# Prasaya/brax

Measured on AMD Instinct MI355X. Metric: env-steps/sec (Ant, 4096 envs/GPU), higher is better.
Workload: dtype f32

## Files before the change

brax_amd/csrc/pbd_eval.hip:

```cpp
#define BX_TU_FAST
#include <hip/hip_runtime.h>
#include <stdint.h>

#include "pbd_dispatch.h"
#include "pbd_kernels.hip"
#include "pbd_launch.h"

namespace bx {

template <int L, int MODE, int F, int M, int EK = EK_ANY>
__global__ void __launch_bounds__(L > 64 ? L : 64) BX_STEP_ATTR
env_eval_policy_kernel(EnvArgs A, PolArgs Q, EvalArgs V) {
  env_step_body<L, MODE, F, M, EK, true, false, true, true>(A, Q, V);
}
template <int L, int MODE, int F, int M, int EK = EK_ANY>
__global__ void __launch_bounds__(L > 64 ? L : 64) __attribute__((amdgpu_waves_per_eu(2)))
env_eval_policy_wide_kernel(EnvArgs A, PolArgs Q, EvalArgs V) {
  env_step_body<L, MODE, F, M, EK, true, false, true, true>(A, Q, V);
}

BX_ENV_FAMILY(EvalPolicyFamily, FAM_EVAL_POLICY, env_eval_policy_kernel, env_eval_policy_wide_kernel)
hipError_t launch_env_eval_policy(int L, int feat, int gw, int tpb, int64_t n_envs, size_t lds,
                                  hipStream_t s, const EnvArgs& a, const PolArgs& q,
                                  const EvalArgs& v, int fold) {
  return launch_env_family<EvalPolicyFamily>(L, feat, gw, tpb, n_envs, lds, s, fold, a, q, v);
}

}
```

brax_amd/csrc/pbd_features.h:

```cpp
#pragma once
#if defined(__HIPCC__)
#include <hip/hip_runtime.h>
#endif

namespace bx {

enum { F_SPH = 1, F_ANGLE = 2, F_CC = 4, F_TW = 8, F_FORCE = 16, F_ALL = 31 };
enum { F_G1 = 32 };
enum { F_X = 64, F_GEN = F_ALL | F_X };
enum { F_JH = 128 };
enum { F_R2 = 256 };
enum { F_C16 = 512 };
enum { F_R2G = 1024 };
enum { F_CCO = 2048 };
enum { F_LEAN = F_CC | F_TW };

constexpr bool cb_feat(int F) {
#if defined(BX_NO_CB)
  return false;
#else
  return (F & F_JH) != 0 && (F & F_G1) != 0 &&
         (F & (F_CC | F_TW | F_R2 | F_C16 | F_FORCE | F_SPH)) == 0;
#endif
}

#if defined(__HIPCC__)
template <int F, int M> __device__ __forceinline__ constexpr int cl_width() {
  return (F & F_C16) ? 16 : M;
}
template <int F> __device__ __forceinline__ bool is_rev(int type) {
  if constexpr ((F & F_SPH) == 0) return true; else return type == 1;
}
template <int F> __device__ __forceinline__ bool is_torque(int type) {
  if constexpr ((F & F_ANGLE) == 0) return true; else return type == 0;
}
template <int F> __device__ __forceinline__ bool is_plane(int fn) {
  if constexpr ((F & F_CCO) != 0) return false;
  else if constexpr ((F & F_CC) == 0) return true; else return fn == 0;
}
template <int F> __device__ __forceinline__ constexpr bool HALF() {
  return (F & F_CCO) != 0 && (F & F_R2G) != 0;
}
template <int F> __device__ __forceinline__ bool is_oneway(int ow) {
  if constexpr ((F & F_CCO) != 0) return false;
  else if constexpr ((F & F_TW) == 0) return true; else return ow != 0;
}
#endif

enum { LIM_G0 = 0, LIM_G1 = 2, LIM_G2 = 4, LIM_SLOTS = 6 };

enum { EK_ANY = 0, EK_ANT = 1, EK_HUM = 2, EK_CHEETAH = 3, EK_PUSHER = 4 };

enum { MODE_GLOBAL = 0, MODE_SINGLE = 1, MODE_LDS = 2, MODE_MULTI = 3 };

}
```

brax_amd/csrc/pbd_kernels.hip:

```cpp
#pragma once
#include <hip/hip_runtime.h>
#include <stdint.h>
#include <stdlib.h>
#include <string.h>

#include <type_traits>

#include "pbd_features.h"
#include "pbd_launch.h"
#include "pbd_layout.h"
#include "pbd_math.h"
#include "pbd_stamps.h"

namespace bx {

struct Cst {
  const uint32_t* __restrict__ w;
  __device__ __forceinline__ int i(int off) const { return (int)w[off]; }
  __device__ __forceinline__ float f(int off) const { return __uint_as_float(w[off]); }
  __device__ __forceinline__ v3 f3(int off) const { return mk(f(off), f(off + 1), f(off + 2)); }
};

struct BodyC {
  float mass;
// ... 469 lines not shown
}

__device__ __forceinline__ void seg_seg(v3 a0, v3 a1, v3 b0, v3 b1, v3& ba, v3& bb) {
  v3 da = a1 - a0;
  float la = safe_norm(da);
  la += 1e-6f * (float)(la == 0.f);
  da = da / la;
  float hla = la * 0.5f;
  v3 db = b1 - b0;
  float lb = safe_norm(db);
  lb += 1e-6f * (float)(lb == 0.f);
  db = db / lb;
  float hlb = lb * 0.5f;
  v3 am = a0 + da * hla, bm = b0 + db * hlb;
  v3 tr = am - bm;
  float dadb = dot(da, db), datr = dot(da, tr), dbtr = dot(db, tr);
  float den = 1.f - dadb * dadb;
  float ota = (-datr + dadb * dbtr) / (den + 1e-6f);
  float otb = dbtr + ota * dadb;
  float ta = clampf(ota, -hla, hla), tb = clampf(otb, -hlb, hlb);
  ba = am + da * ta;
  bb = bm + db * tb;
  v3 na, nb;
  float d1 = seg_point(a0, a1, bb, na);
  float d2 = seg_point(b0, b1, ba, nb);
  if (d1 < d2) ba = na; else bb = nb;
}

template <int F>
__device__ __forceinline__ void contact_gen(const RowC& R, const QP& a, const QP& b, v3& pos, v3& vel, v3& n,
                            float& pen) {
  if (is_plane<F>(R.fn)) {
  BX_IEEE_IN_CONTACT
    v3 e = a.pos + rotate(R.a_end, a.rot);
    n = rotate(mk(0.f, 0.f, 1.f), b.rot);
    pos = e - n * R.a_rad;
    vel = a.vel + cross(a.ang, pos - a.pos);
    pen = dot(b.pos - pos, n);
    return;
  }
  v3 pa = a.pos + rotate(R.a_pos, a.rot), ea = rotate(R.a_end, a.rot);
  v3 pb = b.pos + rotate(R.b_pos, b.rot), eb = rotate(R.b_end, b.rot);
  v3 a0 = pa + ea, a1 = pa - ea, b0 = pb + eb, b1 = pb - eb;
  v3 ba, bb;
  seg_seg(a0, a1, b0, b1, ba, bb);
  v3 pv = ba - bb;
  float dist = safe_norm(pv);
  n = pv / (1e-6f + dist);
  pen = R.a_rad + R.b_rad - dist + nan_of(dot(pv, pv));
  pos = (ba + bb) / 2.f;
  vel = (a.vel + cross(a.ang, pos - a.pos)) - (b.vel + cross(b.ang, pos - b.pos));
}


__device__ __forceinline__ float pdiv(float a, float b) { return (float)((double)a / (double)b); }

__device__ __noinline__ void heightmap_contact(const Cst& c, const BlobHdr& H, int o, const RowC& R,
                                               const QP& a, const QP& b, v3& pos, v3& vel, v3& n,
                                               float& pen) {
  const float cell = c.f(o + R_X);
  const int off = H.o_hm + c.i(o + R_HM_OFF), M = c.i(o + R_HM_M);
  v3 r = rotate(R.a_end, a.rot);
  pos = a.pos + r;
  vel = a.vel + cross(a.ang, r);
  v3 p = rotate(pos - b.pos, quat_inv(b.rot));
  float u = pdiv(p.x, cell), v = pdiv(p.y, cell);
  float fu = floorf(u), fv = floorf(v);
  int iu = (int)fu, iv = (int)fv;
  bool lower = ((u - fu) + (v - fv)) < 1.f;
  float mu = lower ? -1.f : 1.f;
  int tu[3] = {iu + (lower ? 0 : 1), iu + (lower ? 1 : 0), iu + (lower ? 0 : 1)};
  int tv[3] = {iv + (lower ? 0 : 1), iv + (lower ? 0 : 1), iv + (lower ? 1 : 0)};
  float hh[3];
#pragma unroll
  for (int k = 0; k < 3; k++) {
    int i = tu[k], j = -tv[k];
    i += i < 0 ? M : 0;
    j += j < 0 ? M : 0;
    i = i < 0 ? 0 : (i >= M ? M - 1 : i);
    j = j < 0 ? 0 : (j >= M ? M - 1 : j);
    hh[k] = c.f(off + i * M + j);
  }
  v3 raw = mk(mu * (hh[1] - hh[0]), mu * (hh[2] - hh[0]), cell);
  const float rn = safe_norm(raw);
  v3 n0 = mk(pdiv(raw.x, rn), pdiv(raw.y, rn), pdiv(raw.z, rn));
  v3 p0 = mk((float)tu[0] * cell, (float)tv[0] * cell, hh[0]);
  pen = dot(p0 - p, n0);
  n = rotate(n0, b.rot);
}

__device__ __noinline__ void clipped_contact(const Cst& c, int o, const RowC& R, const QP& a,
                                             const QP& b, v3& pos, v3& vel, v3& n, float& pen) {
  v3 e = a.pos + rotate(R.a_end, a.rot);
  v3 nb = rotate(c.f3(o + R_X), b.rot);
  float ndir = dot(a.pos, nb) > 0.f ? 1.f : -1.f;
  n = nb * ndir;
  pos = e - n * R.a_rad;
  vel = a.vel + cross(a.ang, pos - a.pos);
  v3 pt = rotate(c.f3(o + R_X + 9), b.rot) + b.pos;
  pen = dot(pt - pos, n);
  v3 nx = rotate(c.f3(o + R_X + 3), b.rot), ny = rotate(c.f3(o + R_X + 6), b.rot);
  const float hx = c.f(o + R_X + 12), hy = c.f(o + R_X + 13);
  v3 nn = n * ndir;
  v3 yn = cross(nn, nx), xn = -cross(nn, ny);
  bool front = dot(pos - (pt + nx * hx), xn) > 1e-6f;
  front |= dot(pos - (pt - nx * hx), -xn) > 1e-6f;
// ... 1707 lines not shown
    float c0 = 0.f;
#pragma unroll
    for (int k = 0; k < M; k++) {
      v3 v;
      q4 q;
      float f;
      ld_slot(cslot + (g.e[k] & 0xFFFFFF) * SLOT_STRIDE, v, q, f);
      if (!rot4) q = q4{0.f, q.w, q.x, q.y};
      a0 = a0 + v;
      r0 = r0 + q;
      c0 += f;
    }
    const float d0 = eps + c0;
    a = a0 / d0;
    r = q4{r0.w / d0, r0.x / d0, r0.y / d0, r0.z / d0};
    return;
  }
  const int g0 = g.e[0] >> 24;
  v3 a0 = mk(0.f, 0.f, 0.f), a1 = mk(0.f, 0.f, 0.f);
  q4 r0{0.f, 0.f, 0.f, 0.f}, r1{0.f, 0.f, 0.f, 0.f};
  float c0 = 0.f, c1 = 0.f;
#pragma unroll
  for (int k = 0; k < M; k++) {
    const float* s = cslot + (g.e[k] & 0xFFFFFF) * SLOT_STRIDE;
    float m0 = (g.e[k] >> 24) == g0 ? 1.f : 0.f;
    float m1 = 1.f - m0;
    v3 v;
    q4 q;
    float f;
    ld_slot(s, v, q, f);
    if (!rot4) q = q4{0.f, q.w, q.x, q.y};
    a0 = a0 + v * m0;
    a1 = a1 + v * m1;
    r0 = r0 + q * m0;
    r1 = r1 + q * m1;
    c0 += f * m0;
    c1 += f * m1;
  }
  float d0 = eps + c0, d1 = eps + c1;
  a = a0 / d0 + a1 / d1;
  r = q4{r0.w / d0 + r1.w / d1, r0.x / d0 + r1.x / d1, r0.y / d0 + r1.y / d1,
         r0.z / d0 + r1.z / d1};
}

__device__ __forceinline__ void own_contact(v3 v, q4 q, float f, float eps, v3& a, q4& r) {
  BX_IEEE_IN_CONTACT
  const v3 a0 = mk(0.f, 0.f, 0.f) + v;
  const q4 r0 = q4{0.f, 0.f, 0.f, 0.f} + q;
  const float d0 = eps + (0.f + f);
  a = a0 / d0;
  r = q4{r0.w / d0, r0.x / d0, r0.y / d0, r0.z / d0};
}

__device__ __forceinline__ void vproj(QP& q, v3 ppos, q4 prot, const BodyC& B, float h,
                                      bool bare = false, bool fast = false) {
  BX_IEEE_IN_BODY
  q4 nr = bare ? qnormalize_bare(q.rot) : qnormalize(q.rot, fast);
  const bool nd = !bare && !fast;
  q.vel = mul(nd ? ndiv3(q.pos - ppos, h) : (q.pos - ppos) / h, B.pm);
  q4 dq = quat_mul(nr, quat_inv(prot));
  v3 a = nd ? ndiv3(2.f * mk(dq.x, dq.y, dq.z), h) : 2.f * mk(dq.x, dq.y, dq.z) / h;
  float scl = dq.w >= 0.f ? 1.f : -1.f;
  q.ang = mul(mul(scl * B.rm, a), B.rm);
  q.rot = nr;
}

template <int L, int F, int M, bool FOLD = false, bool NOINFO = false, bool FULL = false>
__device__ void pbd_step_single(const Cst& c, const BlobHdr& H, const Env& E, int lane, bool valid,
                                const float* act, int aw, const Hoist<M, cl_width<F, M>()>& X,
                                v3& icv, v3& ica, v3& iaa) {
  static_assert(!FULL || ((F & F_JH) != 0 && L == 16), "FULL: the 16-lane joint halves");
  const bool hasB = FULL || X.hasB, hasJ = FULL || X.hasJ, hasA = FULL || X.hasA;
#ifdef BX_STAMPS
  unsigned long long st_acc[10] = {0, 0, 0, 0, 0, 0, 0, 0, 0, 0};
  unsigned long long st_last;
  asm volatile("s_memtime %0\n\ts_waitcnt lgkmcnt(0)" : "=s"(st_last)::"memory");
#endif
  const float h = H.h;
  const v3 g = mk(H.gx, H.gy, H.gz);
  constexpr bool JH = (F & F_JH) != 0;
  constexpr bool JLH = (F & F_SPH) == 0;
  const uint4* LIP = (F & F_SPH) != 0 ? E.jlim + lane : nullptr;
  const int jx = lane & 7;
  const bool child = (lane & 8) != 0;
  static_assert(!JH || (L == 16 && (F & F_SPH) == 0), "joint halves: revolute joints at 16 lanes");
  constexpr bool JB = FOLD && JH && (F & F_C16) == 0;
  constexpr bool CB = JB && cb_feat(F);
  const int bi = JB ? X.S.body : lane;
  float* myqp = E.qp + bi * QP_STRIDE;
  QP q;
  if (hasB) q = ldqp(myqp);
  if constexpr (JB) {
    if (lane < H.N) {
      const float* r = E.qp + lane * QP_STRIDE;
      const QP o = ldqp(r);
      st_slot(E.prev + lane * PREV_STRIDE, o.pos, o.rot, 0.f);
      st_rb(E.rb + lane * RB_STRIDE, o.pos, o.vel, o.ang);
      float* acc = E.acc + lane * ACC_STRIDE;
      st3(acc + ACC_ICV, mk(0.f, 0.f, 0.f));
      st3(acc + ACC_ICA, mk(0.f, 0.f, 0.f));
      st3(acc + ACC_IAA, mk(0.f, 0.f, 0.f));
    }
  }
  icv = mk(0.f, 0.f, 0.f);
  ica = mk(0.f, 0.f, 0.f);
  iaa = mk(0.f, 0.f, 0.f);
  float al[3] = {0.f, 0.f, 0.f};
  if (hasA && valid) {
#pragma unroll
    for (int l = 0; l < 3; l++) {
      int ai = X.A.idx[l];
      al[l] = act[take_idx(ai, aw)] * (ai >= 0 ? 1.f : 0.f);
    }
  }
  v3 fv = mk(0.f, 0.f, 0.f), fa = mk(0.f, 0.f, 0.f);
  if constexpr ((F & F_FORCE) != 0) {
    if (hasB) body_forces(c, H, lane, act, aw, valid, fv, fa);
  }
  for (int it = 0; it < H.substeps / 2; it++) {
    v3 ppos = q.pos;
    q4 prot = q.rot;
    v3 dpa_last = mk(0.f, 0.f, 0.f);
#if defined(BX_SUB_UNROLL)
#pragma unroll
#else
#pragma unroll 1
#endif
    for (int sub = 0; sub < 2; sub++) {
      ppos = q.pos;
      prot = q.rot;
      if (!CB && sub == 1 && hasB) st_slot(E.prev + bi * PREV_STRIDE, ppos, prot, 0.f);
      if constexpr (JH) {
        const int jb = X.S.body;
        if constexpr (JB) {
          const JointC& Jc = X.J;
          const v3 oa = xh3(q.ang);
          const v3 tqd = -1.f * Jc.damping * (sel3(child, oa, q.ang) - sel3(child, q.ang, oa));
          if (hasA) act_torque_half<F>(X.J, X.JL, X.S, X.A, E, al, jx, child, q.rot, &tqd);
        } else if constexpr (FOLD) {
          const JointC& Jc = X.J;
          const v3 tqd = -1.f * Jc.damping * (ld_ang(E.qp + Jc.bp * QP_STRIDE) - ld_ang(E.qp + Jc.bc * QP_STRIDE));
          if (hasA) act_torque_half<F>(X.J, X.JL, X.S, X.A, E, al, jx, child, ld_rot(E.qp + jb * QP_STRIDE), &tqd);
        } else {
        if (hasA) act_torque_half<F>(X.J, X.JL, X.S, X.A, E, al, jx, child, ld_rot(E.qp + jb * QP_STRIDE));
        }
        if (!FOLD && hasJ) {
// ... 49 lines not shown
          const QP o = JB ? q : ldqp(E.qp + X.S.body * QP_STRIDE);
          v3 dpo;
          q4 dro;
          joint_apply_half(Jc, X.JL, X.S, child, o, dpo, dro);
          st_slot(E.jslot + (child ? E.nJ + jx : jx) * SLOT_STRIDE, dpo, dro, 0.f);
        }
      } else if (hasJ) {
        const JointC& Jc = X.J;
        QP p = ldqp(E.qp + Jc.bp * QP_STRIDE), cq = ldqp(E.qp + Jc.bc * QP_STRIDE);
        v3 dpp, dcp;
        q4 dpr, dcr;
        joint_apply<F, L>(Jc, p, cq, dpp, dpr, dcp, dcr, JLH, X.JL, LIP);
        st_slot(E.jslot + lane * SLOT_STRIDE, dpp, dpr, 0.f);
        st_slot(E.jslot + (E.nJ + lane) * SLOT_STRIDE, dcp, dcr, 0.f);
      }
      phase_sync();
      BX_STAMP(2);
      if (hasB) {
        v3 dp = mk(0.f, 0.f, 0.f);
        q4 dr{0.f, 0.f, 0.f, 0.f};
#pragma unroll
        for (int k = 0; k < M; k++) {
          v3 v;
          q4 r;
          float f;
          ld_slot(E.jslot + X.jl.e[k] * SLOT_STRIDE, v, r, f);
          dp = dp + v;
          dr = dr + r;
        }
        q.pos = q.pos + mul(dp, X.B.pm);
        q.rot = q4{q.rot.w + dr.w * X.B.qm.w, q.rot.x + dr.x * X.B.qm.x, q.rot.y + dr.y * X.B.qm.y,
                   q.rot.z + dr.z * X.B.qm.z};
        if (sub == 0) vproj(q, ppos, prot, X.B, h, JB);
        if (!JB || (!CB && sub == 1)) stqp(myqp, q);
      }
      phase_sync();
      BX_STAMP(3);
    }
    constexpr bool R2 = (F & F_R2) != 0;
    v3 cpos = mk(0.f, 0.f, 0.f), cn = mk(0.f, 0.f, 0.f);
    float pen = 0.f, dl = 0.f;
    v3 cpos2 = mk(0.f, 0.f, 0.f), cn2 = mk(0.f, 0.f, 0.f);
    float pen2 = 0.f, dl2 = 0.f;
    constexpr bool RG = (F & F_R2G) != 0;
    constexpr int F1 = RG ? (F & ~(F_CC | F_TW)) : F;
    constexpr int F2 = RG ? (F | F_CCO) : F;
    const v3 z3 = mk(0.f, 0.f, 0.f);
    const q4 z4{0.f, 0.f, 0.f, 0.f};
    if constexpr (CB) {
      const RowC& R = X.R;
      v3 oap = z3, oav = z3, oaa = z3, rop = z3, rov = z3, roa = z3;
      q4 oar = z4;
      if (hasB) {
        const QP b = ldqp(E.qp + R.b * QP_STRIDE);
        v3 pbp, obp, cvel;
        q4 pbr, obr;
        float unused;
        ld_slot(E.prev + R.b * PREV_STRIDE, pbp, pbr, unused);
        contact_gen<F>(R, q, b, cpos, cvel, cn, pen);
        dl = position_contact<F>(R, q, b, ppos, prot, pbp, pbr, cpos, cn, pen, oap, oar, obp, obr);
        if (!X.hasR) {
          oap = z3;
          oar = z4;
        }
        held(oap);
        held(oar);
      }
      BX_STAMP(4);
      if (hasB) {
        v3 dp;
        q4 dr;
        own_contact(oap, oar, nonzero3(oap), 1e-6f, dp, dr);
        q.pos = q.pos + mul(dp, X.B.pm);
        q.rot = q4{q.rot.w + dr.w * X.B.qm.w, q.rot.x + dr.x * X.B.qm.x, q.rot.y + dr.y * X.B.qm.y,
                   q.rot.z + dr.z * X.B.qm.z};
        rop = q.pos;
        rov = q.vel;
        roa = q.ang;
        vproj(q, ppos, prot, X.B, h, JB);
        held(q.pos); held(q.rot); held(q.vel); held(q.ang);
        held(rop); held(rov); held(roa);
        held(cpos); held(cn); held(pen); held(dl);
      }
      BX_STAMP(5);
      if (hasB) {
        const QP b = ldqp(E.qp + R.b * QP_STRIDE);
        v3 rbp, rbv, rba, obv, oba;
        ld_rb(E.rb + R.b * RB_STRIDE, rbp, rbv, rba);
        velocity_contact<F>(R, h, q, b, rop, rov, roa, rbp, rbv, rba, cpos, cn, pen, dl, oav, oaa,
                            obv, oba);
        if (!X.hasR) {
          oav = z3;
          oaa = z3;
        }
        held(oav);
        held(oaa);
      }
      BX_STAMP(6);
      if (hasB) {
        v3 dv;
        q4 da;
        own_contact(oav, q4{0.f, oaa.x, oaa.y, oaa.z}, nonzero3(oav), 1e-6f, dv, da);
        v3 dav = mk(da.x, da.y, da.z);
        q.vel = mul(q.vel + dv, X.B.pm);
        q.ang = mul(q.ang + dav, X.B.rm);
        stqp(myqp, q);
        icv = icv + dv;
        ica = ica + dav;
        iaa = iaa + dpa_last;
      }
      phase_sync();
      BX_STAMP(7);
      continue;
    }
    auto pos_pass = [&](auto fc, const RowC& R, int r, v3& cpos, v3& cn, float& pen, float& dl) {
      constexpr int FS = decltype(fc)::value;
      QP a = ldqp(E.qp + R.a * QP_STRIDE), b = ldqp(E.qp + R.b * QP_STRIDE);
      v3 cvel;
      bool far = false;
      if constexpr (NOINFO && (FS & F_CCO) != 0) {
        const v3 d = (a.pos + rotate(R.a_pos, a.rot)) - (b.pos + rotate(R.b_pos, b.rot));
        const float reach =
            (norm(R.a_end) + norm(R.b_end) + R.a_rad + R.b_rad) * 1.00001f + 1e-4f;
        const float dd = dot(d, d);
        far = dd > reach * reach && !is_nan(dd);
      }
      if (far) {
        cpos = z3;
        cn = z3;
        pen = -1.f;
      } else {
        contact_gen<FS>(R, a, b, cpos, cvel, cn, pen);
      }
      if constexpr (HALF<FS>()) {
        const bool sb = (lane & 8) != 0;
        v3 pop, op = z3;
        q4 por, orr = z4;
        float unused;
        ld_slot(E.prev + (sb ? R.b : R.a) * PREV_STRIDE, pop, por, unused);
        if (is_nan(pen)) {
          const float pz = nan_of(pen);
// ... 1361 lines not shown
  }
}
template <int L, bool POP = false>
__device__ __forceinline__ float* policy_eval(const PolArgs& Q, const float* W, const float* pobs,
                                              float* b0, float* b1, int lane, int64_t el, int64_t e,
                                              bool valid, int t, int aw, int64_t n_envs, int head = 0) {
  const float* hin = pobs;
  if (Q.mean) {
    for (int i = lane; i < Q.width[0]; i += L) {
      const float o = pobs[i];
      const float r = (o - Q.mean[i]) / Q.std[i];
      b0[i] = is_nan(o) ? o : r;
    }
    hin = b0;
    esync<L>();
  }
  float* hout = hin == b0 ? b1 : b0;
  for (int l = 0; l < Q.n_layers; l++) {
    const int n_in = Q.width[l], n_out = Q.width[l + 1];
    pol_layer<L>(W, hin, hout, n_in, n_out, lane, l + 1 < Q.n_layers ? Q.act_fn : -1);
    W += (n_in + 1) * n_out;
    esync<L>();
    hin = hout;
    hout = hin == b0 ? b1 : b0;
  }
  if constexpr (POP) {
    if (head == 1) return const_cast<float*>(hin);
  }
  const bool has_scale = Q.width[Q.n_layers] >= 2 * aw;
  for (int a = lane; a < aw; a += L) {
    const float loc = hin[a];
    float scale = 1.f, eps = 0.f;
    if (has_scale) scale = pol_softplus(hin[aw + a]) + Q.min_std;
    if (!Q.det)
      eps = normal_at(Q.seed, Q.offset + (uint64_t)t * Q.step + ((uint64_t)el * (uint64_t)aw + (uint64_t)a) * 2u);
    const float raw = Q.det ? loc : fmaf(scale, eps, loc);
    const float act = pol_tanh(raw);
    const float lp = -0.5f * eps * eps - 0.91893853320467274178f - logf(scale) -
                     2.f * (0.69314718055994530942f - raw - pol_softplus(-2.f * raw));
    hout[a] = act;
    hout[aw + a] = lp;
    if (valid && Q.raw_out) Q.raw_out[((int64_t)t * n_envs + e) * aw + a] = raw;
  }
  esync<L>();
  if (lane == 0 && valid && Q.logp_out) {
    float s = 0.f;
    for (int a = 0; a < aw; a++) s += hout[aw + a];
    Q.logp_out[(int64_t)t * n_envs + e] = s;
  }
  return hout;
}

template <int L, int MODE, int F, int M, int EK = EK_ANY, bool PK = false, bool ONE = false,
          bool POL = false, bool EVL = false, bool POP = false>
__device__ __forceinline__ void env_step_body(const EnvArgs& A, const PolArgs& Q = PolArgs{},
                                              const EvalArgs& V = EvalArgs{},
                                              const PopArgs& N = PopArgs{}) {
  static_assert(!EVL || (PK && !ONE), "the evaluation kernels run on the packed K-step layout");
  static_assert(!POP || (POL && EVL), "the population kernels are evaluation kernels with a policy");
  BX_KSTAMP_DECL
  extern __shared__ __attribute__((aligned(16))) float smem[];
  constexpr bool EARLY = PK && ONE && MODE == MODE_SINGLE;
  f32x4 eq0 = {0.f, 0.f, 0.f, 0.f}, eq1 = eq0, eq2 = eq0;
  float eq3 = 0.f;
  if constexpr (EARLY) {
    const int64_t es = A.in.qp.pos.env_stride;
    const int nb = (int)(es >> 4);
    const int ln = (int)(threadIdx.x % L);
    const int64_t ee = (int64_t)blockIdx.x * (blockDim.x / L) + threadIdx.x / L;
    const float* qs = A.in.qp.pos.ptr + (ee < A.n_envs ? ee : 0) * es + (int64_t)(ln < nb ? ln : 0) * 16;
    eq0 = ld4a(qs);
    eq1 = ld4a(qs + 4);
    eq2 = ld4a(qs + 8);
    eq3 = qs[12];
  }
  float ed = 0.f, est = 0.f, ea0 = 0.f, ea1 = 0.f;
  if constexpr (EARLY) {
    const int ln = (int)(threadIdx.x % L);
    const int64_t ee = (int64_t)blockIdx.x * (blockDim.x / L) + threadIdx.x / L;
    const int64_t eel = ee < A.n_envs ? ee : 0;
    ed = A.in.done[eel];
    if (A.in.steps) est = A.in.steps[eel];
    const int aw0 = (int)A.act_width;
    constexpr int C0 = L < 64 ? L : 64;
    if (!A.draw && aw0 > 0 && ln < C0) {
      const float* ar = A.act + eel * A.act_stride;
      ea0 = ar[ln < aw0 ? ln : aw0 - 1];
      if (aw0 > C0) ea1 = ar[C0 + ln < aw0 ? C0 + ln : aw0 - 1];
    }
  }
  BlobHdr H = ONE ? A.hdr : *reinterpret_cast<const BlobHdr*>(A.blob);
  Cst c{A.blob};
  float* ebase = stage_constants<MODE>(A.blob, H, smem, c);
  constexpr bool S = MODE == MODE_SINGLE;
  const int lane = threadIdx.x % L;
  const int le = threadIdx.x / L;
  const int64_t e = (int64_t)blockIdx.x * (blockDim.x / L) + le;
  const bool valid = e < A.n_envs;
  Hoist<M, cl_width<F, M>()> X;
  constexpr bool JBK = S && (F & F_JH) != 0 && EK != EK_ANY && (F & F_C16) == 0;
  if constexpr (S && ONE)
    load_hoist<M, (F & F_JH) != 0, (F & F_R2) != 0, cl_width<F, M>(), JBK, JBK && cb_feat(F)>(
        A.lane_img, H, lane, X);
  Env E = carve(ebase + le * H.env_words, H);
  zero_slots(E, H, lane);
  BX_PSTAMP(5);
  const bx_env_params& P = A.P;
// ... 43 lines not shown
    const int nm = P.n_metrics;
    ev = smem + V.lds_off + le * V.words;
    em = ev + nm + 3;
    if (lane == 0)
      for (int k = 0; k < nm + 3; k++)
        ev[k] = (V.in && valid) ? V.in[k * A.n_envs + e] : (k == nm + 1 ? 1.f : 0.f);
  }
  float* mom = nullptr;
  if constexpr (POP) {
    float* pp = smem + N.lds_off + le * N.words;
    const int nw = 2 * P.obs_size + 1;
    if (N.mom_out) {
      mom = pp;
      for (int i = lane; i < nw; i += L) mom[i] = (N.mom_in && valid) ? N.mom_in[e * nw + i] : 0.f;
    }
    if (N.stage) {
      float* row = pp + N.row_off;
      for (int i = lane * 4; i < Q.n_params; i += L * 4) st4a(row + i, ld4a(pw + i));
      pw = row;
    }
    esync<L>();
  }
  if (!POL && aw > 0 && lane < C) a0 = drw ? draw_at(0, lane < aw ? lane : aw - 1) : (EARLY ? ea0 : arow_g[lane < aw ? lane : aw - 1]);
  BX_PSTAMP(7);
  if constexpr (S) {
    float qv[13];
    if constexpr (EARLY) {
#pragma unroll
      for (int k = 0; k < 4; k++) {
        qv[k] = eq0[k];
        qv[4 + k] = eq1[k];
        qv[8 + k] = eq2[k];
      }
      qv[12] = eq3;
    } else {
      load_qp_regs(A.in.qp, el, lane < H.N ? lane : 0, qv);
    }
    if (lane < H.N) {
      float* s = E.qp + lane * QP_STRIDE;
#pragma unroll
      for (int k = 0; k < 13; k++) s[k] = valid ? qv[k] : (k == 3 ? 1.f : 0.f);
    }
  } else {
    for (int b = lane; b < H.N; b += L) {
      if (valid) {
        load_qp_global(A.in.qp, e, b, E.qp + b * QP_STRIDE);
      } else {
        float* s = E.qp + b * QP_STRIDE;
        for (int k = 0; k < 13; k++) s[k] = k == 3 ? 1.f : 0.f;
      }
    }
  }
  BX_PSTAMP(8);
  const int nst = ONE ? 1 : (A.n_steps > 1 ? A.n_steps : 1);
  for (int t = 0; t < nst; t++) {
  const bool last = !EVL || t == nst - 1;
  const float* act = (valid && !drw) ? A.act + e * A.act_stride + t * A.act_step : nullptr;
  if constexpr (POP) {
    if (mom) {
      const int no = P.obs_size;
      const float w = ev[P.n_metrics + 1];
      for (int i = lane; i < no; i += L) {
        const float o = pobs[i];
        const float d = Q.mean ? o - Q.mean[i] : o;
        float q = d * d;
        asm("" : "+v"(q));
        mom[i] += w * d;
        mom[no + i] += w * q;
      }
      if (lane == 0) mom[2 * no] += w;
    }
  }
  if constexpr (POL) {
    pact = policy_eval<L, POP>(Q, pw, pobs, pb0, pb1, lane, el, e, valid, t, aw, A.n_envs, POP ? N.head : 0);
    esync<L>();
  } else if (t > 0) {
    if (drw) {
      if (aw > 0 && lane < C) a0 = draw_at(t, lane < aw ? lane : aw - 1);
    } else {
      arow_g = A.act + el * A.act_stride + t * A.act_step;
      if (aw > 0 && lane < C) a0 = arow_g[lane < aw ? lane : aw - 1];
    }
  }
  bx_env_state O;
  float* blk = nullptr;
  if constexpr (PK) {
    const int64_t B = A.n_envs;
    blk = EVL ? A.out.qp.pos.ptr : A.out.qp.pos.ptr + t * A.out_step;
    O.obs = blk + B * H.N * 16;
    O.reward = O.obs + B * P.obs_size;
    O.done = O.reward + B;
    O.steps = O.reward + 2 * B;
    O.truncation = O.reward + 3 * B;
    O.metrics = P.n_metrics > 0 ? O.reward + 4 * B : nullptr;
    O.rng = A.out.rng ? A.out.rng + (EVL ? 0 : t * A.rng_step) : nullptr;
  } else {
    O = A.out;
    if (t > 0) {
      const int64_t os = t * A.out_step;
      O.qp.pos.ptr += os; O.qp.rot.ptr += os; O.qp.vel.ptr += os; O.qp.ang.ptr += os;
      O.obs += os; O.reward += os; O.done += os;
      if (O.metrics) O.metrics += os;
      if (O.steps) O.steps += os;
      if (O.truncation) O.truncation += os;
      if (O.rng) O.rng += t * A.rng_step;
    }
// ... 65 lines not shown
      st3(E.red + 36, ld3(E.qp + (int)P.coef[0] * QP_STRIDE));
    float near0 = 0.f, dist0 = 0.f;
    if (KIND_IS(BX_ENV_PUSHER)) {
      v3 tip = ld3(E.qp + (int)P.coef[0] * QP_STRIDE), obj = ld3(E.qp + (int)P.coef[1] * QP_STRIDE);
      v3 goal = ld3(E.qp + (int)P.coef[2] * QP_STRIDE);
      near0 = -norm(obj - tip);
      dist0 = -norm(obj - goal);
    }
    const float* sact = valid ? E.arow : nullptr;
    int saw = aw;
    float* xact = E.xact;
    if (KIND_IS(BX_ENV_REACHERANGLE)) {
      if (valid && lane < aw) xact[lane] = P.coef[2 + lane] + P.coef[4 + lane] * ((act[lane] + 1.f) / 2.f);
      sact = valid ? xact : nullptr;
    } else if (KIND_IS(BX_ENV_SWIMMER)) {
      const float* q = E.qp + lane * QP_STRIDE;
      q4 rot{0.f, 0.f, 0.f, 0.f};
      v3 vel = mk(0.f, 0.f, 0.f);
      if (lane < 3) {
        rot = q4{q[3], q[4], q[5], q[6]};
        vel = ld3(q + 7);
        v3 lv = rotate(vel, quat_inv(rot));
        float l = lane == 0 ? lv.x : (lane == 1 ? lv.y : lv.z);
        E.red[60 + lane] = P.coef[3 + lane] * fabsf(l) * l;
      }
      esync<L>();
      if (lane < 3 && valid) {
        v3 f = vel * P.coef[2] - mk(E.red[60], E.red[61], E.red[62]);
        f = rotate(f, rot);
        xact[aw + 3 * lane] = clampf(f.x, -5.f, 5.f);
        xact[aw + 3 * lane + 1] = clampf(f.y, -5.f, 5.f);
        xact[aw + 3 * lane + 2] = clampf(f.z, -5.f, 5.f);
      }
      if (valid && lane < aw) xact[lane] = act[lane];
      sact = valid ? xact : nullptr;
      saw = aw + 9;
    } else if (KIND_IS(BX_ENV_GRASP)) {
      for (int i = lane; i < aw; i += L)
        if (valid) xact[i] = P.act_map[i] + P.act_map[aw + i] * ((act[i] + 1.f) / 2.f);
      esync<L>();
      if (lane == 0 && valid) {
        float* pp = E.qp + (int)P.coef[0] * QP_STRIDE;
        v3 palm = ld3(pp);
        v3 d = mk(xact[aw - 3], xact[aw - 2], xact[aw - 1]) - palm;
        float nrm = norm(d);
        float scl = nrm > 2.f ? 2.f / nrm : 1.f;
        st3(pp, palm + scl * d * .15f);
      }
      sact = valid ? xact : nullptr;
    }
    esync<L>();
    if constexpr (S) {
      v3 ica, iaa;
      pbd_step_single<L, F, M, EK != EK_ANY, true>(c, H, E, lane, valid, sact, saw, X, icv, ica, iaa);
    } else if (H.spring) {
      spring_step<L, F>(c, H, E, lane, valid, sact, saw);
    } else {
      pbd_step<L, F>(c, H, E, lane, valid, sact, saw);
    }
    BX_KSTAMP(11);
    env_observe<L, EK>(c, H, E, lane, kind, P.obs_flags, P.obs_size, act, aw,
                   (valid && (POL || last)) ? (POL ? pobs : O.obs + e * P.obs_size) : nullptr, P.coef, S ? &X.J : nullptr,
                   (S && !JBK) ? &X.B : nullptr, (S && EK == EK_HUM) ? &X.A : nullptr);
    BX_KSTAMP(12);
    float ccs = 0.f;
    if constexpr (S && EK == EK_ANT && L == 16) {
      const v3 cv = mk(clip1(icv.x), clip1(icv.y), clip1(icv.z));
      ccs = row_sum16(X.own ? cv.x * cv.x + cv.y * cv.y + cv.z * cv.z : 0.f);
    }
    if (lane == 0 && valid) {
      const float dt = H.dt;
      float* m = EVL ? (P.n_metrics > 0 ? em : nullptr) : (O.metrics ? O.metrics + e * P.n_metrics : nullptr);
      v3 p1 = ld3(E.qp);
      float reward = 0.f;
      if (KIND_IS(BX_ENV_ANT)) {
        v3 vel = (p1 - pos0) / dt;
        float fwd = vel.x;
        float z = p1.z;
        float healthy = in_range_or_nan(z, P.coef[4], P.coef[5]) ? 1.f : 0.f;
        bool term = P.coef[6] != 0.f;
        float hr = term ? P.coef[3] : P.coef[3] * healthy;
        float ctrl = P.coef[1] * sq;
        float cs = ccs;
        if constexpr (!(S && EK == EK_ANT && L == 16))
          for (int b = 0; b < H.N; b++)
            for (int k = 0; k < 3; k++) {
              float cv = clip1(E.acc[b * ACC_STRIDE + ACC_ICV + k]);
              cs += cv * cv;
            }
        float ccost = P.coef[2] * cs;
        reward = fwd + hr - ctrl - ccost;
        done = term ? 1.f - healthy : 0.f;
        if (m) {
          m[0] = norm(p1); m[1] = fwd; m[2] = -ccost; m[3] = -ctrl; m[4] = fwd;
          m[5] = hr; m[6] = p1.x; m[7] = vel.x; m[8] = p1.y; m[9] = vel.y;
        }
      } else if (KIND_IS(BX_ENV_HALFCHEETAH)) {
        float v0 = (p1.x - pos0.x) / dt;
        float fwd = P.coef[0] * v0;
        float ctrl = P.coef[1] * sq;
        reward = fwd - ctrl;
        if (m) { m[0] = -ctrl; m[1] = fwd; m[2] = p1.x; m[3] = v0; }
      } else if (KIND_IS(BX_ENV_HUMANOID)) {
        v3 com1 = ld3(E.red + 32);
        v3 v = (com1 - com0) / dt;
        float fwd = P.coef[0] * v.x;
        float z = p1.z;
// ... 163 lines not shown
    if (lane == 0 && last) {
      O.reward[e] = reward_sum;
      O.done[e] = done;
      if (O.steps) O.steps[e] = steps;
      if (O.truncation) O.truncation[e] = trunc;
    }
    if constexpr (EVL) {
      if (lane == 0) {
        const int nm = P.n_metrics;
        const float active = ev[nm + 1];
        if (active != 0.f) ev[nm + 2] = steps;
        for (int k = 0; k < nm; k++) ev[k] += em[k] * active;
        if constexpr (POP) ev[nm] += (reward_sum - N.reward_shift) * active;
        else ev[nm] += reward_sum * active;
        ev[nm + 1] = active * (1.f - done);
        if (last) {
          for (int k = 0; k < nm; k++) O.metrics[e * nm + k] = em[k];
          for (int k = 0; k < nm + 3; k++) V.out[k * A.n_envs + e] = ev[k];
        }
      }
    }
    if constexpr (POP) {
      if (last && mom) {
        const int nw = 2 * P.obs_size + 1;
        for (int i = lane; i < nw; i += L) N.mom_out[e * nw + i] = mom[i];
      }
    }
    if (reset_now) {
      for (int b = lane; b < H.N; b += L) {
        float tmp[13];
        load_qp_global(P.first_qp, e, b, tmp);
        if (last) store_out_qp(b, tmp);
        if (t + 1 < nst) {
          float* s = E.qp + b * QP_STRIDE;
#pragma unroll
          for (int k = 0; k < 13; k++) s[k] = tmp[k];
        }
      }
      for (int i = lane; i < P.obs_size; i += L) {
        const float fo = P.first_obs[e * P.obs_size + i];
        if (last) O.obs[e * P.obs_size + i] = fo;
        if constexpr (POL) pobs[i] = fo;
      }
    } else if (last) {
      for (int b = lane; b < H.N; b += L) store_out_qp(b, E.qp + b * QP_STRIDE);
      if constexpr (POL)
        for (int i = lane; i < P.obs_size; i += L) O.obs[e * P.obs_size + i] = pobs[i];
    }
  }
  done_in = done;
  steps_in = steps;
  rng_c += (uint32_t)reps;
  esync<L>();
  }
  BX_KSTAMP(14);
}



template <int L, int MODE, int F, int M, int EK = EK_ANY>
__global__ void __launch_bounds__(L > 64 ? L : 64) BX_STEP_ATTR env_step_kernel(EnvArgs A) {
  env_step_body<L, MODE, F, M, EK>(A);
}

}
```

brax_amd/csrc/pbd_policy.hip:

```cpp
#define BX_TU_FAST
#include <hip/hip_runtime.h>
#include <stdint.h>

#include "pbd_dispatch.h"
#include "pbd_kernels.hip"
#include "pbd_launch.h"

namespace bx {

template <int L, int MODE, int F, int M, int EK = EK_ANY>
__global__ void __launch_bounds__(L > 64 ? L : 64) BX_STEP_ATTR
env_policy_rollout_kernel(EnvArgs A, PolArgs Q) {
  env_step_body<L, MODE, F, M, EK, true, false, true>(A, Q);
}
template <int L, int MODE, int F, int M, int EK = EK_ANY>
__global__ void __launch_bounds__(L > 64 ? L : 64) __attribute__((amdgpu_waves_per_eu(2)))
env_policy_rollout_wide_kernel(EnvArgs A, PolArgs Q) {
  env_step_body<L, MODE, F, M, EK, true, false, true>(A, Q);
}

BX_ENV_FAMILY(PolicyFamily, FAM_POLICY, env_policy_rollout_kernel, env_policy_rollout_wide_kernel)
hipError_t launch_env_policy_single(int L, int feat, int gw, int tpb, int64_t n_envs, size_t lds,
                                    hipStream_t s, const EnvArgs& a, const PolArgs& q, int fold) {
  return launch_env_family<PolicyFamily>(L, feat, gw, tpb, n_envs, lds, s, fold, a, q);
}

__global__ void normal_slabs_kernel(float* out, int64_t slab_n, int64_t n, uint64_t seed,
                                    uint64_t offset, uint64_t slab_stride,
                                    const int64_t* __restrict__ epoch, uint64_t epoch_stride) {
  int64_t i = (int64_t)blockIdx.x * blockDim.x + threadIdx.x;
  if (i >= n) return;
  const uint64_t e = epoch ? (uint64_t)epoch[0] : 0ull;
  const int64_t sl = i / slab_n, j = i - sl * slab_n;
  out[i] = normal_at(seed, offset + e * epoch_stride + (uint64_t)sl * slab_stride + 2u * (uint64_t)j);
}
hipError_t launch_normal_slabs(float* out, int64_t slab_n, int64_t n_slabs, uint64_t seed,
                               uint64_t offset, uint64_t slab_stride, const int64_t* epoch,
                               uint64_t epoch_stride, hipStream_t s) {
  const int64_t n = slab_n * n_slabs;
  dim3 grid((unsigned)((n + 255) / 256));
  hipLaunchKernelGGL(normal_slabs_kernel, grid, dim3(256), 0, s, out, slab_n, n, seed, offset,
                     slab_stride, epoch, epoch_stride);
  return hipGetLastError();
}

}
```

brax_amd/csrc/pbd_pop.hip:

```cpp
#define BX_TU_FAST
#include <hip/hip_runtime.h>
#include <stdint.h>

#include "pbd_dispatch.h"
#include "pbd_kernels.hip"
#include "pbd_launch.h"

namespace bx {

template <int L, int MODE, int F, int M, int EK = EK_ANY>
__global__ void __launch_bounds__(L > 64 ? L : 64) BX_STEP_ATTR
env_eval_pop_kernel(EnvArgs A, PolArgs Q, EvalArgs V, PopArgs N) {
  env_step_body<L, MODE, F, M, EK, true, false, true, true, true>(A, Q, V, N);
}
template <int L, int MODE, int F, int M, int EK = EK_ANY>
__global__ void __launch_bounds__(L > 64 ? L : 64) __attribute__((amdgpu_waves_per_eu(2)))
env_eval_pop_wide_kernel(EnvArgs A, PolArgs Q, EvalArgs V, PopArgs N) {
  env_step_body<L, MODE, F, M, EK, true, false, true, true, true>(A, Q, V, N);
}

BX_ENV_FAMILY(PopulationFamily, FAM_POPULATION, env_eval_pop_kernel, env_eval_pop_wide_kernel)
hipError_t launch_env_eval_population(int L, int feat, int gw, int tpb, int64_t n_envs, size_t lds,
                                      hipStream_t s, const EnvArgs& a, const PolArgs& q,
                                      const EvalArgs& v, const PopArgs& n, int fold) {
  return launch_env_family<PopulationFamily>(L, feat, gw, tpb, n_envs, lds, s, fold, a, q, v, n);
}

}
```

Baseline: 198.0 million.

## Freeze static ground body state in registers for CB Ant step kernels

For kernels where the contact partner is a single frozen body (ground plane), this loads the partner's pose and plane normal once before the step loop and holds them in registers. It reloads them only after a reset. Contact generation then uses a specialized plane routine instead of re-reading qp, prev and rb slots for body b every substep. Per-body prev slot writes and the acceleration records are skipped or zeroed once up front. This removes repeated global loads and generic contact dispatch, at the cost of extra live registers and the assumption that body b never moves. The wide kernel variants opt out.

```diff
diff --git a/brax_amd/csrc/pbd_eval.hip b/brax_amd/csrc/pbd_eval.hip
--- a/brax_amd/csrc/pbd_eval.hip
+++ b/brax_amd/csrc/pbd_eval.hip
@@ -16,7 +16,7 @@
 template <int L, int MODE, int F, int M, int EK = EK_ANY>
 __global__ void __launch_bounds__(L > 64 ? L : 64) __attribute__((amdgpu_waves_per_eu(2)))
 env_eval_policy_wide_kernel(EnvArgs A, PolArgs Q, EvalArgs V) {
-  env_step_body<L, MODE, F, M, EK, true, false, true, true>(A, Q, V);
+  env_step_body<L, MODE, F, M, EK, true, false, true, true, false, false>(A, Q, V);
 }
 
 BX_ENV_FAMILY(EvalPolicyFamily, FAM_EVAL_POLICY, env_eval_policy_kernel, env_eval_policy_wide_kernel)
diff --git a/brax_amd/csrc/pbd_features.h b/brax_amd/csrc/pbd_features.h
--- a/brax_amd/csrc/pbd_features.h
+++ b/brax_amd/csrc/pbd_features.h
@@ -21,6 +21,14 @@
 #else
   return (F & F_JH) != 0 && (F & F_G1) != 0 &&
          (F & (F_CC | F_TW | F_R2 | F_C16 | F_FORCE | F_SPH)) == 0;
+#endif
+}
+
+constexpr bool cbh_feat(int F) {
+#if defined(BX_NO_CBH)
+  return false;
+#else
+  return cb_feat(F);
 #endif
 }
 
diff --git a/brax_amd/csrc/pbd_kernels.hip b/brax_amd/csrc/pbd_kernels.hip
--- a/brax_amd/csrc/pbd_kernels.hip
+++ b/brax_amd/csrc/pbd_kernels.hip
@@ -545,6 +545,16 @@
   vel = (a.vel + cross(a.ang, pos - a.pos)) - (b.vel + cross(b.ang, pos - b.pos));
 }
 
+__device__ __forceinline__ void contact_gen_plane(const RowC& R, const QP& a, v3 bpos, v3 nb,
+                                                  v3& pos, v3& vel, v3& n, float& pen) {
+  BX_IEEE_IN_CONTACT
+  v3 e = a.pos + rotate(R.a_end, a.rot);
+  n = nb;
+  pos = e - n * R.a_rad;
+  vel = a.vel + cross(a.ang, pos - a.pos);
+  pen = dot(bpos - pos, n);
+}
+
 
 __device__ __forceinline__ float pdiv(float a, float b) { return (float)((double)a / (double)b); }
 
@@ -2358,6 +2368,25 @@
   r = q4{r0.w / d0, r0.x / d0, r0.y / d0, r0.z / d0};
 }
 
+struct FrozenB {
+  QP b;
+  v3 n;
+};
+__device__ __forceinline__ FrozenB load_frozen(const float* rec) {
+  FrozenB Z;
+  Z.b = ldqp(rec);
+  Z.n = rotate(mk(0.f, 0.f, 1.f), Z.b.rot);
+  return Z;
+}
+__device__ __forceinline__ void init_frozen_records(const BlobHdr& H, const Env& E, int lane) {
+  if (lane < H.N) {
+    float* acc = E.acc + lane * ACC_STRIDE;
+    st3(acc + ACC_ICV, mk(0.f, 0.f, 0.f));
+    st3(acc + ACC_ICA, mk(0.f, 0.f, 0.f));
+    st3(acc + ACC_IAA, mk(0.f, 0.f, 0.f));
+  }
+}
+
 __device__ __forceinline__ void vproj(QP& q, v3 ppos, q4 prot, const BodyC& B, float h,
                                       bool bare = false, bool fast = false) {
   BX_IEEE_IN_BODY
@@ -2371,11 +2400,13 @@
   q.rot = nr;
 }
 
-template <int L, int F, int M, bool FOLD = false, bool NOINFO = false, bool FULL = false>
+template <int L, int F, int M, bool FOLD = false, bool NOINFO = false, bool FULL = false,
+          bool CBH = false>
 __device__ void pbd_step_single(const Cst& c, const BlobHdr& H, const Env& E, int lane, bool valid,
                                 const float* act, int aw, const Hoist<M, cl_width<F, M>()>& X,
-                                v3& icv, v3& ica, v3& iaa) {
+                                v3& icv, v3& ica, v3& iaa, const FrozenB Z = FrozenB{}) {
   static_assert(!FULL || ((F & F_JH) != 0 && L == 16), "FULL: the 16-lane joint halves");
+  static_assert(!CBH || (FOLD && (F & F_JH) != 0 && (F & F_C16) == 0 && cb_feat(F)), "CBH: a CB kernel");
   const bool hasB = FULL || X.hasB, hasJ = FULL || X.hasJ, hasA = FULL || X.hasA;
 #ifdef BX_STAMPS
   unsigned long long st_acc[10] = {0, 0, 0, 0, 0, 0, 0, 0, 0, 0};
@@ -2397,7 +2428,7 @@
   QP q;
   if (hasB) q = ldqp(myqp);
   if constexpr (JB) {
-    if (lane < H.N) {
+    if (!CBH && lane < H.N) {
       const float* r = E.qp + lane * QP_STRIDE;
       const QP o = ldqp(r);
       st_slot(E.prev + lane * PREV_STRIDE, o.pos, o.rot, 0.f);
@@ -2553,12 +2584,20 @@
       v3 oap = z3, oav = z3, oaa = z3, rop = z3, rov = z3, roa = z3;
       q4 oar = z4;
       if (hasB) {
-        const QP b = ldqp(E.qp + R.b * QP_STRIDE);
+        QP b;
         v3 pbp, obp, cvel;
         q4 pbr, obr;
-        float unused;
-        ld_slot(E.prev + R.b * PREV_STRIDE, pbp, pbr, unused);
-        contact_gen<F>(R, q, b, cpos, cvel, cn, pen);
+        if constexpr (CBH) {
+          b = Z.b;
+          pbp = b.pos;
+          pbr = b.rot;
+          contact_gen_plane(R, q, b.pos, Z.n, cpos, cvel, cn, pen);
+        } else {
+          b = ldqp(E.qp + R.b * QP_STRIDE);
+          float unused;
+          ld_slot(E.prev + R.b * PREV_STRIDE, pbp, pbr, unused);
+          contact_gen<F>(R, q, b, cpos, cvel, cn, pen);
+        }
         dl = position_contact<F>(R, q, b, ppos, prot, pbp, pbr, cpos, cn, pen, oap, oar, obp, obr);
         if (!X.hasR) {
           oap = z3;
@@ -2585,9 +2624,17 @@
       }
       BX_STAMP(5);
       if (hasB) {
-        const QP b = ldqp(E.qp + R.b * QP_STRIDE);
+        QP b;
         v3 rbp, rbv, rba, obv, oba;
-        ld_rb(E.rb + R.b * RB_STRIDE, rbp, rbv, rba);
+        if constexpr (CBH) {
+          b = Z.b;
+          rbp = b.pos;
+          rbv = b.vel;
+          rba = b.ang;
+        } else {
+          b = ldqp(E.qp + R.b * QP_STRIDE);
+          ld_rb(E.rb + R.b * RB_STRIDE, rbp, rbv, rba);
+        }
         velocity_contact<F>(R, h, q, b, rop, rov, roa, rbp, rbv, rba, cpos, cn, pen, dl, oav, oaa,
                             obv, oba);
         if (!X.hasR) {
@@ -4055,7 +4102,7 @@
 }
 
 template <int L, int MODE, int F, int M, int EK = EK_ANY, bool PK = false, bool ONE = false,
-          bool POL = false, bool EVL = false, bool POP = false>
+          bool POL = false, bool EVL = false, bool POP = false, bool ZH = true>
 __device__ __forceinline__ void env_step_body(const EnvArgs& A, const PolArgs& Q = PolArgs{},
                                               const EvalArgs& V = EvalArgs{},
                                               const PopArgs& N = PopArgs{}) {
@@ -4205,6 +4252,20 @@
     }
   }
   BX_PSTAMP(8);
+  constexpr bool CBH = ZH && JBK && cbh_feat(F);
+  FrozenB Z{};
+  auto freeze = [&]() {
+    if (X.hasB) {
+      Z = load_frozen(E.qp + X.R.b * QP_STRIDE);
+      held(Z.b.pos); held(Z.b.rot); held(Z.b.vel); held(Z.b.ang);
+      held(Z.n);
+    }
+  };
+  if constexpr (CBH) {
+    esync<L>();
+    init_frozen_records(H, E, lane);
+    freeze();
+  }
   const int nst = ONE ? 1 : (A.n_steps > 1 ? A.n_steps : 1);
   for (int t = 0; t < nst; t++) {
   const bool last = !EVL || t == nst - 1;
@@ -4376,7 +4437,8 @@
     esync<L>();
     if constexpr (S) {
       v3 ica, iaa;
-      pbd_step_single<L, F, M, EK != EK_ANY, true>(c, H, E, lane, valid, sact, saw, X, icv, ica, iaa);
+      pbd_step_single<L, F, M, EK != EK_ANY, true, false, CBH>(c, H, E, lane, valid, sact, saw, X, icv,
+                                                               ica, iaa, Z);
     } else if (H.spring) {
       spring_step<L, F>(c, H, E, lane, valid, sact, saw);
     } else {
@@ -4646,6 +4708,9 @@
   steps_in = steps;
   rng_c += (uint32_t)reps;
   esync<L>();
+  if constexpr (CBH) {
+    if (valid && reset_now && t + 1 < nst) freeze();
+  }
   }
   BX_KSTAMP(14);
 }
diff --git a/brax_amd/csrc/pbd_policy.hip b/brax_amd/csrc/pbd_policy.hip
--- a/brax_amd/csrc/pbd_policy.hip
+++ b/brax_amd/csrc/pbd_policy.hip
@@ -16,7 +16,7 @@
 template <int L, int MODE, int F, int M, int EK = EK_ANY>
 __global__ void __launch_bounds__(L > 64 ? L : 64) __attribute__((amdgpu_waves_per_eu(2)))
 env_policy_rollout_wide_kernel(EnvArgs A, PolArgs Q) {
-  env_step_body<L, MODE, F, M, EK, true, false, true>(A, Q);
+  env_step_body<L, MODE, F, M, EK, true, false, true, false, false, false>(A, Q);
 }
 
 BX_ENV_FAMILY(PolicyFamily, FAM_POLICY, env_policy_rollout_kernel, env_policy_rollout_wide_kernel)
diff --git a/brax_amd/csrc/pbd_pop.hip b/brax_amd/csrc/pbd_pop.hip
--- a/brax_amd/csrc/pbd_pop.hip
+++ b/brax_amd/csrc/pbd_pop.hip
@@ -16,7 +16,7 @@
 template <int L, int MODE, int F, int M, int EK = EK_ANY>
 __global__ void __launch_bounds__(L > 64 ? L : 64) __attribute__((amdgpu_waves_per_eu(2)))
 env_eval_pop_wide_kernel(EnvArgs A, PolArgs Q, EvalArgs V, PopArgs N) {
-  env_step_body<L, MODE, F, M, EK, true, false, true, true, true>(A, Q, V, N);
+  env_step_body<L, MODE, F, M, EK, true, false, true, true, true, false>(A, Q, V, N);
 }
 
 BX_ENV_FAMILY(PopulationFamily, FAM_POPULATION, env_eval_pop_kernel, env_eval_pop_wide_kernel)
```

Measured after the change: 200.0 million (median of 6 runs). 1.0% higher.
